# PacificBiosciences/ccs

Measured on AMD Instinct MI355X. Metric: ZMWs/sec (HiFi reads/sec), 10-pass x 10 kb synthetic, higher is better.
Workload: dtype f32

## Files before the change

### ccs_amd/csrc/ccsx_api.cpp

```cpp
#include <hip/hip_runtime.h>

#include <algorithm>
#include <cmath>
#include <cstdio>
#include <cstdlib>
#include <cstring>
#include <initializer_list>
#include <mutex>
#include <string>
#include <vector>

#include "ccsx.h"
#include "ccsx_internal.h"
#include "ccsx_kernels.h"
#include "refine_core.h"

#define HIPTRY(expr)                                                                                           \
    do {                                                                                                       \
        hipError_t e_ = (expr);                                                                                \
        if (e_ != hipSuccess) {                                                                                \
            ccsx_set_error(std::string(#expr) + ": " + hipGetErrorString(e_));                                 \
            return -2;                                                                                         \
        }                                                                                                      \
    } while (0)
// ... 1410 lines not shown
}
int ccsx_submit_hd_requests(ccsx_handle h, const ccsx_batch *b, ccsx_results *res, const ccsx_requests *rq, const ccsx_hd_request *hd, ccsx_ticket *ticket)
{
    Wants W;
    if (hd_requests_wants(rq, hd, b, __func__, &W)) return -1;
    return submit_impl(h, b, res, ticket, CCSX_RUN_FUSED, nullptr, nullptr, 0, W, __func__);
}
int ccsx_submit_hd(ccsx_handle h, const ccsx_batch *b, ccsx_results *res, const ccsx_extras *ex, const ccsx_hd_request *hd, ccsx_ticket *ticket)
{
    const ccsx_requests rq = {ex, nullptr, nullptr, nullptr, nullptr, {nullptr, nullptr, nullptr}};
    Wants W;
    if (hd_requests_wants(&rq, hd, b, __func__, &W)) return -1;
    return submit_impl(h, b, res, ticket, CCSX_RUN_FUSED, nullptr, nullptr, 0, W, __func__);
}
int ccsx_submit_handoff(ccsx_handle h, const ccsx_batch *b, ccsx_results *res, const ccsx_requests *rq, const ccsx_handoff_request *ho, ccsx_ticket *ticket)
{
    Wants W;
    if (requests_wants(rq, b, __func__, &W, ho) || (!ho && refuse(__func__, "null handoff request"))) return -1;
    return submit_impl(h, b, res, ticket, CCSX_RUN_FUSED, nullptr, nullptr, 0, W, __func__);
}
int ccsx_submit_barcodes(ccsx_handle h, const ccsx_batch *b, ccsx_results *res, const ccsx_requests *rq, const ccsx_barcode_request *bc, ccsx_ticket *ticket)
{
    Wants W;
    if ((!bc && refuse(__func__, "null barcode request")) || (!b && refuse(__func__, "null argument")) || requests_wants(rq, b, __func__, &W, nullptr, bc)) return -1;
    return submit_impl(h, b, res, ticket, CCSX_RUN_FUSED, nullptr, nullptr, 0, W, __func__);
}
static int represent_wants(ccsx_handle h, const ccsx_batch *b, const ccsx_requests *rq, const ccsx_represent_request *rp, const char *fn, Wants *W)
{
    if (!rp) return refuse(fn, "null represent request");
    if (!h || !b) return refuse(fn, "null argument");
    if (ccsx_represent_check(rp, b, &h->opts, fn)) return -1;
    if (rq && rq->coverage && rq->coverage->gate != 0) return refuse(fn, "the represent request is not combined with the coverage gate");
    if (requests_wants(rq, b, fn, W)) return -1;
    W->represent_req = *rp; W->represent = true;
    return 0;
}
int ccsx_submit_represent(ccsx_handle h, const ccsx_batch *b, ccsx_results *res, const ccsx_requests *rq, const ccsx_represent_request *rp, ccsx_ticket *ticket)
{
    Wants W;
    if (represent_wants(h, b, rq, rp, __func__, &W)) return -1;
    return submit_impl(h, b, res, ticket, CCSX_RUN_FUSED, nullptr, nullptr, 0, W, __func__);
}
int ccsx_submit_draft(ccsx_handle h, const ccsx_batch *b, ccsx_drafts *drafts, ccsx_ticket *ticket)
{
    return submit_impl(h, b, nullptr, ticket, CCSX_RUN_DRAFT, drafts, nullptr, 0, Wants{}, __func__);
}
int ccsx_submit_polish(ccsx_handle h, const ccsx_batch *b, const ccsx_drafts *drafts, ccsx_results *res, uint32_t flags, ccsx_ticket *ticket)
{
    return submit_impl(h, b, res, ticket, CCSX_RUN_POLISH, nullptr, drafts, flags, Wants{}, __func__);
}
int ccsx_draft_batch(ccsx_handle h, const ccsx_batch *b, ccsx_drafts *drafts)
{
    ccsx_ticket t;
    if (int rc = ccsx_submit_draft(h, b, drafts, &t)) return rc;
    return ccsx_wait(h, t);
}
int ccsx_polish_batch(ccsx_handle h, const ccsx_batch *b, const ccsx_drafts *drafts, ccsx_results *res, uint32_t flags)
{
    ccsx_ticket t;
    if (int rc = ccsx_submit_polish(h, b, drafts, res, flags, &t)) return rc;
    return ccsx_wait(h, t);
}

int ccsx_submit_refine(ccsx_handle h, const ccsx_batch *b, const ccsx_results *base, const int32_t *backbone, const ccsx_refine_tiles *tiles, ccsx_results *res,
                       ccsx_refine_report *report, ccsx_ticket *ticket)
{
    RefineReq rf;
    if (refine_request_check(b, base, backbone, tiles, report, &rf, __func__)) return -1;
    return submit_impl(h, b, res, ticket, CCSX_RUN_POLISH, nullptr, nullptr, CCSX_QV_ONLY, Wants{}, __func__, &rf);
}
int ccsx_refine_batch(ccsx_handle h, const ccsx_batch *b, const ccsx_results *base, const int32_t *backbone, const ccsx_refine_tiles *tiles, ccsx_results *res,
                      ccsx_refine_report *report)
{
    ccsx_ticket t;
    if (int rc = ccsx_submit_refine(h, b, base, backbone, tiles, res, report, &t)) return rc;
    return ccsx_wait(h, t);
}

static Slot *slot_of(ccsx_handle h, ccsx_ticket t)
{
    if (!h || t < 0) return nullptr;
    Slot &S = h->slot[t % CCSX_SLOTS];
    return S.ticket == t ? &S : nullptr;
}

int ccsx_wait(ccsx_handle h, ccsx_ticket ticket)
{
    Slot *S = slot_of(h, ticket);
    if (!S) { ccsx_set_error("ccsx_wait: unknown or recycled ticket"); return -1; }
    HIPTRY(hipSetDevice(h->device));
    return retire(h, *S);
}

int ccsx_poll(ccsx_handle h, ccsx_ticket ticket)
{
    Slot *S = slot_of(h, ticket);
    if (!S) { ccsx_set_error("ccsx_poll: unknown or recycled ticket"); return -1; }
    const hipError_t e = hipEventQuery(S->ev_done);
    if (e == hipErrorNotReady) return 0;
    if (e != hipSuccess) { ccsx_set_error(std::string("ccsx_poll: ") + hipGetErrorString(e)); return -2; }
    HIPTRY(hipSetDevice(h->device));
    return retire(h, *S) ? -2 : 1;
}

int ccsx_ticket_timings(ccsx_handle h, ccsx_ticket ticket, ccsx_timings *t)
{
    Slot *S = slot_of(h, ticket);
    if (!S || !t || !(S->ran || S->tm_ok)) { ccsx_set_error("ccsx_ticket_timings: unknown ticket"); return -1; }
    if (S->tm_ok) { *t = S->tm; return 0; }
    HIPTRY(hipSetDevice(h->device));
    return slot_timings(h, *S, t);
}

static int upload_impl(ccsx_handle h, const ccsx_batch *b, const Wants &W)
{
    if (!h) { ccsx_set_error("ccsx_upload: null handle"); return -1; }
    HIPTRY(hipSetDevice(h->device));
    for (auto &S : h->slot) if (int rc = retire(h, S)) return rc;
    Slot &S = h->slot[0];
    S.ticket = -1;
    const int rc = stage(h, S, b, h->s_comp, W);
    if (rc) { S.staged = false; return rc; }
    S.mode = CCSX_RUN_FUSED;
    HIPTRY(hipStreamSynchronize(h->s_comp));
    h->last = 0;
    return 0;
}

int ccsx_upload(ccsx_handle h, const ccsx_batch *b) { return upload_impl(h, b, Wants{}); }

int ccsx_run(ccsx_handle h)
{
    if (!h || !h->slot[0].staged || h->slot[0].mode != CCSX_RUN_FUSED) { ccsx_set_error("ccsx_run: no batch uploaded for the fused path: call ccsx_upload first"); return -1; }
    HIPTRY(hipSetDevice(h->device));
    h->last = 0;
    return launch(h, h->slot[0]);
}

int ccsx_sync(ccsx_handle h)
{
    if (!h) return -1;
    HIPTRY(hipSetDevice(h->device));
    HIPTRY(hipStreamSynchronize(h->s_draft));
    HIPTRY(hipStreamSynchronize(h->s_comp));
    Slot &S = h->slot[h->last];
#ifdef CCSX_PROFILE_PHASES
    if (S.staged && S.ran) {
        unsigned long long ph[16];
        HIPTRY(hipMemcpy(ph, S.P.phase, sizeof(ph), hipMemcpyDeviceToHost));
        static const char *nm[8] = {"prologue", "tables+lanes", "chunk plan", "fill", "score", "select/apply", "qv+store", "validity+list"};
        unsigned long long tot = 0;
        for (int i = 0; i < 8; ++i) tot += ph[i];
        for (int i = 0; i < 8; ++i) std::fprintf(stderr, "[ccsx phase] %-14s %6.2f %%  (%llu cycles)\n", nm[i], tot ? 100.0 * ph[i] / tot : 0.0, ph[i]);
        static const char *pn[6] = {"thr setup+read", "thr traceback", "thr ids+zero", "thr records", "thr order", "thr col records"};
        unsigned long long pt = 0;
        for (int i = 8; i < 14; ++i) pt += ph[i];
        for (int i = 8; i < 14; ++i) std::fprintf(stderr, "[ccsx phase] %-14s %6.2f %%  (%llu cycles)\n", pn[i - 8], pt ? 100.0 * ph[i] / pt : 0.0, ph[i]);
    }
#endif
#ifdef CCSX_DEBUG_CHECKS
    if (S.staged) {
        int32_t dbg[2] = {0, 0};
        HIPTRY(hipMemcpy(dbg, S.P.debug, 8, hipMemcpyDeviceToHost));
        if (dbg[0]) { ccsx_set_error("device bounds check failed: code " + std::to_string(dbg[0]) + " at kernel line " + std::to_string(dbg[1])); return -3; }
    }
#endif
    (void)S;
    return 0;
}

int ccsx_download(ccsx_handle h, ccsx_results *res)
{
    if (!h || !h->slot[0].ran || h->slot[0].mode != CCSX_RUN_FUSED || !res) { ccsx_set_error("ccsx_download: nothing to download: ccsx_upload + ccsx_run first"); return -1; }
    Slot &S = h->slot[0];
    if (int rc = check_results(S, res, S.P.out_kin != nullptr)) return rc;
    HIPTRY(hipSetDevice(h->device));
    if (int rc = enqueue_download(S, res, h->s_comp)) return rc;
    HIPTRY(hipStreamSynchronize(h->s_comp));
    finish_outputs(S, res, nullptr);
    return 0;
}

int ccsx_consensus_batch(ccsx_handle h, const ccsx_batch *b, ccsx_results *res)
{
    int rc;
    if ((rc = ccsx_upload(h, b))) return rc;
    if ((rc = ccsx_run(h))) return rc;
    if ((rc = ccsx_sync(h))) return rc;
    return ccsx_download(h, res);
}

int ccsx_pileup_rule_version(void) { return 1; }

static int consensus_sync(ccsx_handle h, const ccsx_batch *b, ccsx_results *res, const Wants &W, const char *fn)
{
    if (!h || !b || !res) return refuse(fn, "null argument");
    int rc;
    if ((rc = upload_impl(h, b, W))) return rc;
    Slot &S = h->slot[0];
    if ((rc = check_results(S, res, S.P.out_kin != nullptr)) || (rc = attach(h, S, W, h->s_comp))) return rc;
    HIPTRY(hipStreamSynchronize(h->s_comp));
    if ((rc = ccsx_run(h)) || (rc = ccsx_sync(h)) || (rc = ccsx_download(h, res))) return rc;
    if ((rc = enqueue_wants_download(S, W, h->s_comp))) return rc;
    HIPTRY(hipStreamSynchronize(h->s_comp));
    return 0;
}

int ccsx_consensus_pileup(ccsx_handle h, const ccsx_batch *b, ccsx_results *res, ccsx_pileup *pile)
{
    const ccsx_extras ex = {pile, nullptr, 0, 0};
    Wants W;
    if (build_wants(&ex, nullptr, nullptr, nullptr, nullptr, b, __func__, &W) || (!pile && refuse(__func__, "null argument"))) return -1;
    return consensus_sync(h, b, res, W, __func__);
}

int ccsx_tandem_rule_version(void) { return 1; }

int ccsx_consensus_extras(ccsx_handle h, const ccsx_batch *b, ccsx_results *res, const ccsx_extras *ex)
{
    Wants W;
    if (build_wants(ex, nullptr, nullptr, nullptr, nullptr, b, __func__, &W)) return -1;
    return consensus_sync(h, b, res, W, __func__);
}

int ccsx_consensus_hd_requests(ccsx_handle h, const ccsx_batch *b, ccsx_results *res, const ccsx_requests *rq, const ccsx_hd_request *hd)
{
    Wants W;
    if (hd_requests_wants(rq, hd, b, __func__, &W)) return -1;
    return consensus_sync(h, b, res, W, __func__);
}

int ccsx_consensus_hd(ccsx_handle h, const ccsx_batch *b, ccsx_results *res, const ccsx_extras *ex, const ccsx_hd_request *hd)
{
    const ccsx_requests rq = {ex, nullptr, nullptr, nullptr, nullptr, {nullptr, nullptr, nullptr}};
    Wants W;
    if (hd_requests_wants(&rq, hd, b, __func__, &W)) return -1;
    return consensus_sync(h, b, res, W, __func__);
}

void ccsx_fold_opts_default(ccsx_fold_opts *o)
{
    if (!o) return;
    o->max_occ = 8; o->min_hits = 12; o->min_arm = 200; o->min_span_tenths = 8; o->end_slack = 100;
}

int ccsx_fold_rule_version(void) { return 1; }

int ccsx_consensus_fold(ccsx_handle h, const ccsx_batch *b, ccsx_results *res, const ccsx_extras *ex, const ccsx_fold_request *fold)
{
    Wants W;
    if (build_wants(ex, nullptr, fold, nullptr, nullptr, b, __func__, &W) || (!fold && refuse(__func__, "null request or report"))) return -1;
    return consensus_sync(h, b, res, W, __func__);
}

void ccsx_adapter_opts_default(ccsx_adapter_opts *o)
{
    if (!o) return;
    o->max_dist_pct = 20; o->min_copies = 2; o->max_insert = 100; o->end_slack = 200;
}

int ccsx_adapter_rule_version(void) { return 1; }

int ccsx_adapter_set_default(ccsx_adapter_set *s)
{
    if (!s) { ccsx_set_error("ccsx_adapter_set_default: null argument"); return -1; }
    static const char hairpin[] = "ATCTCTCTCTTTTCCTCCTCCTCCGTTGTTGTTGTTGAGAGAGAT";
    std::memset(s, 0, sizeof *s);
    s->n_adapters = 1; s->len[0] = (int32_t)(sizeof hairpin - 1);
    for (int i = 0; i < s->len[0]; ++i) s->seq[0][i] = (uint8_t)(hairpin[i] == 'A' ? 0 : hairpin[i] == 'C' ? 1 : hairpin[i] == 'G' ? 2 : 3);
    return 0;
}

int ccsx_consensus_screen(ccsx_handle h, const ccsx_batch *b, ccsx_results *res, const ccsx_extras *ex, const ccsx_fold_request *fold, const ccsx_adapter_request *adapters)
{
    Wants W;
    if (build_wants(ex, nullptr, fold, adapters, nullptr, b, __func__, &W)) return -1;
    return consensus_sync(h, b, res, W, __func__);
}

void ccsx_control_opts_default(ccsx_control_opts *o)
{
    if (!o) return;
    o->max_occ = 4; o->min_matched = 30; o->min_ctl_tenths = 5; o->min_draft_tenths = 8;
}

int ccsx_control_rule_version(void) { return 1; }

int ccsx_consensus_control(ccsx_handle h, const ccsx_batch *b, ccsx_results *res, const ccsx_extras *ex, const ccsx_fold_request *fold, const ccsx_adapter_request *adapters,
                           const ccsx_control_request *control)
{
    Wants W;
    if (build_wants(ex, nullptr, fold, adapters, control, b, __func__, &W)) return -1;
    return consensus_sync(h, b, res, W, __func__);
}

void ccsx_coverage_opts_default(ccsx_coverage_opts *o)
{
    if (!o) return;
    o->drop_percent = 50; o->block = 30; o->min_spans = 0; o->max_lost_percent = 50;
}

int ccsx_coverage_rule_version(void) { return 1; }

int ccsx_consensus_requests(ccsx_handle h, const ccsx_batch *b, ccsx_results *res, const ccsx_requests *rq)
{
    Wants W;
    if (requests_wants(rq, b, __func__, &W)) return -1;
    return consensus_sync(h, b, res, W, __func__);
}

// ... 378 lines not shown
```

### ccs_amd/csrc/ccsx_kernels.hip

```cpp
#include <hip/hip_runtime.h>
#include <stdint.h>
#include <cstdio>
#include <cstdlib>

#include "ccsx.h"
#include "ccsx_kernels.h"
#include "wave_ops.h"

#define LANDED(x) asm volatile("" : "+v"(x))

#if (defined(CCSX_EXP_NO_FILL) || defined(CCSX_EXP_NO_SCORE) || defined(CCSX_EXP_ONE_ROUND) || defined(CCSX_EXP_ALL_VALID) || defined(CCSX_EXP_CHEAP_VALIDITY) || \
     defined(CCSX_EXP_NO_ROWS) || defined(CCSX_EXP_NO_SCORE_LOG) || defined(CCSX_EXP_SKIP_ROUND2_SCORE) || defined(CCSX_EXP_NO_QV_EXP) || defined(CCSX_EXP_REPEAT) || defined(CCSX_EXP_NO_BANDMASK) || \
     defined(CCSX_EXP_HOT_PROLOGUE) || defined(CCSX_EXIT_AFTER_PROLOGUE)) && !defined(CCSX_EXPERIMENT)
#error "CCSX_EXP_* / CCSX_EXIT_AFTER_PROLOGUE switches produce wrong results: build them with -DCCSX_EXPERIMENT (never ship such a library)"
#endif
#define CCSX_STR2(x) #x
#define CCSX_STR(x) CCSX_STR2(x)
int ccsx_kernel_is_experiment()
{
#ifdef CCSX_EXPERIMENT
    return 1;
#else
    return 0;
#endif
// ... 599 lines not shown
        const int vb = rec.x & 3;
        const int p0 = rec.y;
        const unsigned long long multim = actm & M_NE0(rec.x & 0xe00);
        const unsigned long long far0m = actm & M_NE0(rec.x & CREC_FAR0);
        const uint32_t slot0 = p0 < 0 ? PRING : (uint32_t)(p0 & (PRING - 1));
        int k0x, k0y, k0z;
        { const uint32_t ka = kinBase + slot0 * 16; k0x = LDS_I32(ka); k0y = LDS_I32(ka + 4); k0z = LDS_I32(ka + 8); }
        if (__builtin_expect(far0m != 0ull, 0)) { if (rec.x & CREC_FAR0) { const int4 t = kinfo[p0]; k0x = t.x; k0y = t.y; k0z = t.z; } LANDED(k0x); LANDED(k0y); LANDED(k0z); }
        int ulo = k0x, ubr = k0z;
        int plo1 = 0, plo2 = 0;
        if (multim) {
            const int np = (rec.x >> 8) & 15;
            const bool act = live && k < n0;
            int bestcm = k0y;
            for (int q = 1; q < CCSX_MAXPRED; ++q) {
                if ((actm & M_SGT(np, q)) == 0ull) break;
                int pq = q == 1 ? rec.z : rec.w;
                if (q >= 3) {
                    if (act && np > q) pq = pxw[(size_t)k * 4 + (q - 3)];
                    LANDED(pq);
                }
                const bool on = act && np > q;
                const bool farq = on && k - pq > PRING;
                const uint32_t ka = kinBase + (on ? (uint32_t)(pq & (PRING - 1)) : (uint32_t)PRING) * 16;
                int qx = LDS_I32(ka), qy = LDS_I32(ka + 4), qz = LDS_I32(ka + 8);
                if (__builtin_expect(M_NE0(farq ? 1 : 0) != 0ull, 0)) { if (farq) { const int4 t = kinfo[pq]; qx = t.x; qy = t.y; qz = t.z; } LANDED(qx); LANDED(qy); LANDED(qz); }
                if (q == 1) plo1 = qx; else if (q == 2) plo2 = qx;
                if (on && qy > bestcm) { bestcm = qy; ulo = qx; ubr = qz; }
            }
        }
        int lo = imed3(ubr + (1 - PB / 2), ulo, ulo + 2);
        lo = lo < hiI ? lo : hiI;
        lo = lo > 0 ? lo : 0;
        if (__builtin_expect((actm & M_UGT(lo - c0, CH16 - PB - 2)) != 0ull, 0)) {
            __syncthreads();
            if (live && k < n0 && (unsigned)(lo - c0) > (unsigned)(CH16 - PB - 2)) {
                c0 = lo - 128 > 0 ? lo - 128 : 0;
                load_read_chunk_m1(sRead[gq], rb, I, rev, c0, l);
            }
            __syncthreads();
        }
        const int r0w = lo + l2;
        int s0, s1;
        {
            const uint32_t idx = (uint32_t)(r0w - c0) & (CH16 - 1);
            const uint32_t wa = readBase + ((idx >> 4) << 2);
            const uint32_t wlo = (uint32_t)LDS_I32(wa), whi = (uint32_t)LDS_I32(wa + 4);
            const uint32_t t = __builtin_amdgcn_alignbit(whi, wlo, (idx & 15u) << 1);
            s0 = (vb == (int)(t & 3u)) ? SC_MATCH : SC_MISMATCH;
            s1 = (vb == (int)((t >> 2) & 3u)) ? SC_MATCH : SC_MISMATCH;
        }
        int b0, b1, m0, m1;
        {
            const int w = imed3(r0w - k0x + 3, 1, PGS - 3);
            const uint32_t src = ringBase + slot0 * (PGS * 4) + ((uint32_t)w << 2);
            int x0 = LDS_I32(src), y0 = LDS_I32(src + 4), y1 = LDS_I32(src + 8);
            if (__builtin_expect(far0m != 0ull, 0)) {
                if (rec.x & CREC_FAR0) {
                    const int32_t *Mu = Mcol + (size_t)p0 * PB;
                    const int o = r0w - k0x - 1;
                    x0 = (unsigned)o < (unsigned)PB ? Mu[o] : NEGV;
                    y0 = (unsigned)(o + 1) < (unsigned)PB ? Mu[o + 1] : NEGV;
                    y1 = (unsigned)(o + 2) < (unsigned)PB ? Mu[o + 2] : NEGV;
                }
                LANDED(x0); LANDED(y0); LANDED(y1);
            }
            const int d0 = x0 + s0, e0 = y0 + SC_DEL, d1 = y0 + s1, e1 = y1 + SC_DEL;
            const bool t0 = e0 > d0, t1 = e1 > d1;
            b0 = t0 ? e0 : d0; m0 = t0 ? 1 : 0;
            b1 = t1 ? e1 : d1; m1 = t1 ? 1 : 0;
        }
        if (multim) {
            const int np = (rec.x >> 8) & 15;
            const bool act = live && k < n0;
            for (int q = 1; q < CCSX_MAXPRED; ++q) {
                if ((actm & M_SGT(np, q)) == 0ull) break;
                const bool on = act && np > q;
                int pq = q == 1 ? rec.z : rec.w, plo = q == 1 ? plo1 : plo2;
                if (q >= 3) {
                    if (on) {
                        pq = pxw[(size_t)k * 4 + (q - 3)];
                        if (k - pq > PRING) plo = kinfo[pq].x; else plo = LDS_I32(kinBase + (uint32_t)(pq & (PRING - 1)) * 16);
                    }
                    LANDED(pq); LANDED(plo);
                }
                const bool farq = on && k - pq > PRING;
                const int off = r0w - plo;
                const int w = imed3(off + 3, 1, PGS - 3);
                const uint32_t src = ringBase + (on ? (uint32_t)(pq & (PRING - 1)) : (uint32_t)PRING) * (PGS * 4) + ((uint32_t)w << 2);
                int x0 = LDS_I32(src), y0 = LDS_I32(src + 4), y1 = LDS_I32(src + 8);
                if (__builtin_expect(M_NE0(farq ? 1 : 0) != 0ull, 0)) {
                    if (farq) {
                        const int32_t *Mu = Mcol + (size_t)pq * PB;
                        const int o = off - 1;
                        x0 = (unsigned)o < (unsigned)PB ? Mu[o] : NEGV;
                        y0 = (unsigned)(o + 1) < (unsigned)PB ? Mu[o + 1] : NEGV;
                        y1 = (unsigned)(o + 2) < (unsigned)PB ? Mu[o + 2] : NEGV;
                    }
                    LANDED(x0); LANDED(y0); LANDED(y1);
                }
                const int mq = q << 1;
                int c;
                c = x0 + s0;     if (on && c > b0) { b0 = c; m0 = mq; }
                c = y0 + SC_DEL; if (on && c > b0) { b0 = c; m0 = mq | 1; }
                c = y0 + s1;     if (on && c > b1) { b1 = c; m1 = mq; }
                c = y1 + SC_DEL; if (on && c > b1) { b1 = c; m1 = mq | 1; }
            }
        }
        { const int c = b0 + SC_INS; if (c > b1) { b1 = c; m1 = 15; } }
        {
            const int S = row_scan_max_i32(b1 + l8);
            const int Sp = __builtin_amdgcn_update_dpp(-(1 << 30), S, DPP_ROW_SHR(1), 0xf, 0xf, false);
            const int c0v = Sp - (l8 - 8 - SC_INS);
            const int c1v = Sp - (l8 - 8 - 2 * SC_INS);
            if (c0v > b0) { b0 = c0v; m0 = 15; }
            if (c1v > b1) { b1 = c1v; m1 = 15; }
        }
        if (r0w > I || b0 < NEGV / 2) b0 = NEGV;
        if (r0w >= I || b1 < NEGV / 2) b1 = NEGV;
        int cm, br;
        {
            const int f = -(1 << 24);
            const int k0_ = ((b0 > f ? b0 : f) * 64) | kRow0, k1_ = ((b1 > f ? b1 : f) * 64) | kRow1;
            const int key = row_allmax_i32(k0_ > k1_ ? k0_ : k1_);
            cm = key >> 6; br = (lo + 63) - (key & 63);
        }
        if (__builtin_expect((actm & M_SGT(lo + PB, I)) != 0ull, 0)) {
            const int e = r0w == I ? b0 : (r0w + 1 == I ? b1 : NEGV);
            const int ev = __builtin_amdgcn_ds_bpermute(bcastAddr, row_scan_max_i32(e));
            if (live && k < n0 && ev > NEGV / 2 && ev > bs) { bs = ev; kend = k; }
        }
        if (live && k < n0) {
            *(int2 *)&sRing[gq][k & (PRING - 1)][4 + l2] = make_int2(b0, b1);
            *mvp = (uint8_t)(m0 | (m1 << 4));
            if (l == 0) {
                sKin[gq][k & (PRING - 1)] = make_int4(lo, cm, br, 0);
                *lop = lo;
            }
            if (__builtin_expect((rec.x & CREC_NEED) != 0, 0)) {
                *(int2 *)Mp = make_int2(b0, b1);
                if (l == 0) *kip = make_int4(lo, cm, br, p0);
            }
        }
    }
#undef M_NE0
#undef M_SLT
#undef M_SGT
#undef M_UGT
#undef LDS_I32
    __threadfence_block();
    if (live && l == 0) { st[ST_KEND] = kend; st[ST_BS] = bs; }
}

__global__ __launch_bounds__(64) __attribute__((amdgpu_waves_per_eu(8, 8))) void k_poa_thread(KParams P, int z0, int pass, int rr, int b0)
{
    const int bx = (int)blockIdx.x + b0;
    __shared__ __attribute__((aligned(16))) uint8_t sMv[TB_BLOCK * POA_MV_BYTES];
    const int lane = threadIdx.x;
    uint32_t *sread = dyn_lds;
    PoaSlot g = poa_slot(P, bx);
    if (z0 + bx >= P.n_zmw) return;
    if (!g.st[ST_LIVE] || !g.st[ST_OK] || rr >= g.st[ST_NPOA]) return;
    TPH_T0();
    const int z = rfl(P.zmw_perm[z0 + bx]);
    const int r0 = rfl(P.read_off[z]);
    const int bb = rfl(g.st[ST_BB]), nreads = rfl(g.st[ST_NREADS]), npoa = rfl(g.st[ST_NPOA]);
    const int r = r0 + (bb + rr < nreads ? bb + rr : bb + rr - nreads);
    const uint8_t *rb = P.bases + P.base_off[r];
    const int I = rfl((int)(P.base_off[r + 1] - P.base_off[r]));
    const int kend = rfl(g.st[ST_KEND]), bsc = rfl(g.st[ST_BS]);
    int32_t *const plog = (P.poa_log && pass < 2 && rr < P.poa_log_stride) ? P.poa_log + ((size_t)(2 * z + pass) * P.poa_log_stride + rr) * CCSX_POA_LOG_WORDS : nullptr;
    auto log_pass = [&](int threaded, int nv) { if (plog && lane == 0) { plog[0] = I; plog[1] = bsc; plog[2] = kend; plog[3] = threaded; plog[4] = nv; } };
    if (kend < 0 || bsc < I) { log_pass(0, g.st[ST_N]); return; }
    const int rev = rfl(((P.flags[r] & 1) != g.st[ST_REV0]) ? 1 : 0);
    const int vcap = rfl(P.vcap[z]);
    const int n0 = rfl(g.st[ST_N]);
    const int par = rfl(g.st[ST_PAR]);
    const int4 *crec = par ? g.crec1 : g.crec0, *pxc = par ? g.px1 : g.px0;
    int4 *crec_nx = par ? g.crec0 : g.crec1, *px_nx = par ? g.px0 : g.px1;
    load_read_packed(sread, rb, I, rev, lane);
    __syncthreads();
    TPH(8);
    {
        int k = kend, i = I;
        int4 kiN = make_int4(0, 0, 0, -1), crN = make_int4(0, -1, -1, -1);
        int kbN = -1;
        uint4 mvN0 = make_uint4(0, 0, 0, 0);
        auto fetch = [&](int kb_) {
            const int kk = kb_ + lane;
            kbN = kb_;
            kiN = make_int4(0, 0, 0, -1); crN = make_int4(0, -1, -1, -1);
            if (kb_ >= 0) {
                if (kk < n0) { crN = crec[kk]; kiN = make_int4(g.loK[kk], 0, 0, crN.y); }
                mvN0 = ((const uint4 *)(g.mvK + (size_t)kb_ * POA_MV_BYTES))[lane];
            }
        };
        fetch((k / TB_BLOCK) * TB_BLOCK);
        while (k >= 0) {
            const int kb = (k / TB_BLOCK) * TB_BLOCK;
            if (kbN != kb) fetch(kb);
            __syncthreads();
            const int4 kiL = kiN, crL = crN;
            const int metaL = crN.x;
            ((uint4 *)sMv)[lane] = mvN0;
            fetch(kb - TB_BLOCK);
            __syncthreads();
            while (k >= kb) {
                int kl = k - kb;
                int mknown;
                {
                    const int kls = kl - lane;
                    const int src = kls & 63;
                    const int lo_s = __shfl(kiL.x, src), pp_s = __shfl(kiL.w, src);
                    const int off = i - lane - lo_s;
                    const bool inb = kls >= 0 && i - lane >= 1 && (unsigned)off < (unsigned)PB;
                    const int m_s = inb ? ((sMv[kls * POA_MV_BYTES + (off >> 1)] >> ((off & 1) << 2)) & 15) : 255;
                    const unsigned long long simple = __ballot(m_s == 0 && pp_s == k - lane - 1);
                    const int R = (simple == ~0ull) ? 64 : __ffsll((long long)~simple) - 1;
                    if (R > 0) {
                        const int meta_s = __shfl(metaL, src);
                        if (lane < R) {
                            const int ir = i - lane - 1;
                            g.pathv[ir] = ((meta_s & 3) == read_base_packed(sread, ir)) ? k - lane : -1;
                        }
                        k -= R; i -= R;
                        if (R >= 64 || k < kb) continue;
                        kl = k - kb;
                    }
                    mknown = rl(m_s, R);
                }
                const int lo_k = rl(kiL.x, kl);
                CHK(i - lo_k >= 0 && i - lo_k < PB && i >= 0, 101);
                const int mo = i - lo_k;
                const int m = mknown != 255 ? mknown : rfl((sMv[kl * POA_MV_BYTES + (mo >> 1)] >> ((mo & 1) << 2)) & 15);
                const int t = m == 15 ? MV_INS : (m & 1), slot = m >> 1;
                CHK(i >= 1 || t == MV_DEL, 102);
                if (t == MV_INS) { if (lane == 0) g.pathv[i - 1] = -1; --i; continue; }
                const int meta = rl(metaL, kl);
                const int np = (meta >> 8) & 15;
                int up;
                if (np == 0) up = -1;
                else if (slot == 0) up = rl(kiL.w, kl);
                else if (slot == 1) up = rl(crL.z, kl);
                else if (slot == 2) up = rl(crL.w, kl);
                else up = rfl(((const int32_t *)pxc)[(size_t)k * 4 + (slot - 3)]);
                if (t == MV_DIAG) {
                    if (lane == 0) g.pathv[i - 1] = ((meta & 3) == read_base_packed(sread, i - 1)) ? k : -1;
                    --i;
                }
                CHK(up < k && up >= -1, 103);
                k = up;
            }
            k = rfl(k); i = rfl(i);
        }
        for (int q = lane; q < i; q += LANES) g.pathv[q] = -1;
    }
    __threadfence_block();
    TPH(9);
    int32_t *cnt = g.bestK;
    auto newpos = [&](int q) -> int { return q + cnt[q]; };
    for (int q = lane; q <= n0; q += LANES) { cnt[q] = 0; g.onpK[q] = 0; }
    __threadfence_block();
    TPH(10);
    int lastEx = -1, nnew = 0;
    for (int c0 = 0; c0 < I; c0 += 2 * LANES) {
        int w[2], wn[2], ex[2];
        bool valid[2], isnew[2], lastOfRun[2];
#pragma unroll
        for (int u = 0; u < 2; ++u) {
            const int i = c0 + u * LANES + lane;
            valid[u] = i < I;
            const int ic = valid[u] ? i : I - 1;
            w[u] = g.pathv[ic];
            wn[u] = g.pathv[ic + 1 < I ? ic + 1 : ic];
        }
#pragma unroll
        for (int u = 0; u < 2; ++u) {
            const int i = c0 + u * LANES + lane;
            isnew[u] = valid[u] && w[u] < 0;
            nnew += __popcll(__ballot(isnew[u]));
            const int incl = wave_scan_max_i32((valid[u] && !isnew[u]) ? i : -1);
            int e = wave_shr1_i32(incl, -1);
            e = e > lastEx ? e : lastEx;
            ex[u] = e;
            const int li = rl(incl, 63);
            lastEx = li > lastEx ? li : lastEx;
            lastOfRun[u] = isnew[u] && ((i + 1 >= I) || (wn[u] >= 0));
        }
        int av[2];
#pragma unroll
        for (int u = 0; u < 2; ++u) av[u] = g.pathv[(lastOfRun[u] && ex[u] >= 0) ? ex[u] : 0];
#pragma unroll
        for (int u = 0; u < 2; ++u) {
            const int i = c0 + u * LANES + lane;
            if (valid[u] && !isnew[u]) g.onpK[w[u]] = 1;
            if (lastOfRun[u]) {
                const int ap = ex[u] >= 0 ? av[u] : -1;
                CHK(ap >= -1 && ap < n0, 106);
                cnt[ap + 1] = i - ex[u];
            }
        }
    }
    nnew = rfl(nnew);
    if (n0 + nnew > vcap) { if (lane == 0) g.st[ST_OK] = 0; log_pass(0, n0); return; }
    __threadfence_block();
    TPH(11);
    int carry = 0;
    for (int c0 = 0; c0 <= n0; c0 += 4 * LANES) {
        int cv[4];
#pragma unroll
        for (int u = 0; u < 4; ++u) { const int q = c0 + u * LANES + lane; cv[u] = cnt[q <= n0 ? q : n0]; }
#pragma unroll
        for (int u = 0; u < 4; ++u) {
            const int q = c0 + u * LANES + lane;
            const int incl = wave_scan_add_i32(q <= n0 ? cv[u] : 0);
            if (q <= n0) cnt[q] = carry + incl;
            carry += rl(incl, 63);
        }
    }
    const int n = n0 + nnew;
    for (int q = lane; q < n; q += LANES) g.needK[q] = 0;
    __threadfence_block();
    auto carry_over = [&](int q, int kn, int4 rec, int4 &pxr) -> int4 {
        const int np = (rec.x >> 8) & 15;
        rec.x &= ~CREC_FAR0;
        if (np > 0) { rec.y = newpos(rec.y); if (kn - rec.y > PRING) { g.needK[rec.y] = 1; rec.x |= CREC_FAR0; } }
        if (np > 1) { rec.z = newpos(rec.z); if (kn - rec.z > PRING) g.needK[rec.z] = 1; }
        if (np > 2) { rec.w = newpos(rec.w); if (kn - rec.w > PRING) g.needK[rec.w] = 1; }
        if (np > 3) {
            pxr = pxc[q];
            for (int e = 3; e < np; ++e) { const int pn = newpos(int4_get(pxr, e - 3)); int4_set(pxr, e - 3, pn); if (kn - pn > PRING) g.needK[pn] = 1; }
        }
        return rec;
    };
    for (int q0 = 0; q0 < n0; q0 += 2 * LANES) {
        int4 rec[2]; int kn[2]; bool go[2];
#pragma unroll
        for (int u = 0; u < 2; ++u) {
            const int q = q0 + u * LANES + lane;
            go[u] = q < n0 && !g.onpK[q < n0 ? q : 0];
            rec[u] = make_int4(0, -1, -1, -1); kn[u] = 0;
            if (go[u]) { rec[u] = crec[q]; kn[u] = newpos(q); }
        }
#pragma unroll
        for (int u = 0; u < 2; ++u) if (go[u]) {
            const int q = q0 + u * LANES + lane;
            int4 pxr = make_int4(-1, -1, -1, -1);
            const int4 r = carry_over(q, kn[u], rec[u], pxr);
            CHK(kn[u] >= 0 && kn[u] < n, 105);
            crec_nx[kn[u]] = r;
            if (((r.x >> 8) & 15) > 3) px_nx[kn[u]] = pxr;
        }
    }
    TPH(12);
    lastEx = -1;
    int prevP = -1;
    for (int c0 = 0; c0 < I; c0 += LANES) {
        const int i = c0 + lane;
        const bool valid = i < I;
        const int w = g.pathv[valid ? i : I - 1];
        const bool isnew = valid && w < 0;
        const int incl = wave_scan_max_i32((valid && !isnew) ? i : -1);
        int ex = wave_shr1_i32(incl, -1);
        ex = ex > lastEx ? ex : lastEx;
        { const int li = rl(incl, 63); lastEx = li > lastEx ? li : lastEx; }
        const int av = g.pathv[(isnew && ex >= 0) ? ex : 0];
        int4 rec = make_int4(0, -1, -1, -1);
        if (valid && !isnew) rec = crec[w];
        const int qa = valid ? (isnew ? (ex >= 0 ? av : 0) : w) : 0;
        int P = newpos(qa);
        if (isnew) P = (ex >= 0 ? P + 1 : 0) + (i - ex - 1);
        if (!valid) P = -1;
        int Pp = wave_shr1_i32(P, prevP);
        prevP = rl(P, 63);
        if (valid) {
            CHK(P >= 0 && P < n, 104);
            int4 pxr = make_int4(-1, -1, -1, -1);
            bool pxdirty = false;
            if (isnew) rec = make_int4(read_base_packed(sread, i) | ((Pp >= 0 ? 1 : 0) << 8) | (1 << CREC_NREADS_SHIFT), Pp, -1, -1);
            else {
                rec = carry_over(w, P, rec, pxr);
                rec.x += 1 << CREC_NREADS_SHIFT;
                if (Pp >= 0) {
                    const int np = (rec.x >> 8) & 15;
                    bool found = false;
                    if (np > 0) found |= rec.y == Pp;
                    if (np > 1) found |= rec.z == Pp;
                    if (np > 2) found |= rec.w == Pp;
                    for (int e = 3; e < np; ++e) found |= int4_get(pxr, e - 3) == Pp;
                    if (!found && np < CCSX_MAXPRED) {
                        if (np == 0) rec.y = Pp; else if (np == 1) rec.z = Pp; else if (np == 2) rec.w = Pp; else { int4_set(pxr, np - 3, Pp); pxdirty = true; }
                        rec.x += 1 << 8;
                        if (P - Pp > PRING) { g.needK[Pp] = 1; if (np == 0) rec.x |= CREC_FAR0; }
                    }
                }
            }
            crec_nx[P] = rec;
            if (((rec.x >> 8) & 15) > 3 || pxdirty) px_nx[P] = pxr;
        }
    }
    __threadfence_block();
    if (lane == 0) { g.st[ST_N] = n; g.st[ST_NADDED] += 1; g.st[ST_PAR] ^= 1; }
    log_pass(1, n);
    (void)npoa;
    TPH(13);
}

__global__ __launch_bounds__(64) __attribute__((amdgpu_waves_per_eu(8, 8))) void k_poa_finish(KParams P, int z0, int pass, int b0)
{
    const int bx = (int)blockIdx.x + b0;
    const int lane = threadIdx.x;
    PoaSlot g = poa_slot(P, bx);
    if (z0 + bx >= P.n_zmw) return;
    if (!g.st[ST_LIVE]) return;
    const int z = rfl(P.zmw_perm[z0 + bx]);
    const int ok = rfl(g.st[ST_OK]), n = rfl(g.st[ST_N]), nadded = rfl(g.st[ST_NADDED]);
    const int4 *crec = g.st[ST_PAR] ? g.crec1 : g.crec0;
    const int32_t *pxw = (const int32_t *)(g.st[ST_PAR] ? g.px1 : g.px0);
    int Ld = 0, nw = 0, stat = -1;
    if (ok && n > 0) {
        int kbest = -1, sb = NEGV, best_prev = 0;
        for (int kb = 0; kb < n; kb += LANES) {
            const int kkL = kb + lane;
            int4 cL = make_int4(0, -1, -1, -1);
            if (kkL < n) cL = crec[kkL];
            const int nblk = (n - kb) < LANES ? (n - kb) : LANES;
            const int npL = (cL.x >> 8) & 15;
            const int wL = kkL < n ? 2 * ((cL.x >> CREC_NREADS_SHIFT) & 127) - nadded : 0;
            const int Pw = wave_scan_add_i32(wL);
            const bool headL = kkL < n && (lane == 0 || npL != 1 || cL.y != kkL - 1);
            unsigned long long heads = __ballot(headL);
            const unsigned long long headmask = heads;
            int hb = 0, bpv = kkL - 1;
            while (heads) {
                const int j = (int)__ffsll((long long)heads) - 1;
                heads &= heads - 1;
                const int k = kb + j;
                const int np = rl(npL, j);
                int b = 0, p = -1;
                for (int q = 0; q < np; ++q) {
                    int pu;
                    if (q < 3) pu = q == 0 ? rl(cL.y, j) : (q == 1 ? rl(cL.z, j) : rl(cL.w, j));
                    else pu = rfl(pxw[(size_t)k * 4 + (q - 3)]);
                    CHK(pu >= 0 && pu < k, 108);
                    int bu;
                    if (pu >= kb) {
                        const int pj = pu - kb;
                        const int hd = 63 - __clzll((long long)(headmask & ((2ull << pj) - 1ull)));
                        bu = rl(hb, hd) + rl(Pw, pj) - rl(Pw, hd);
                    } else bu = pu == kb - 1 ? best_prev : rfl(g.bestK[pu]);
                    if (bu > b) { b = bu; p = pu; }
                }
                const int bv = b + rl(wL, j);
                if (lane == j) { hb = bv; bpv = p; }
            }
            const int hdL = 63 - __clzll((long long)(headmask & ((2ull << lane) - 1ull)));
            int myBest = __shfl(hb, hdL) + Pw - __shfl(Pw, hdL);
            const unsigned long long nonpos = __ballot(kkL < n && myBest <= 0);
            if ((nonpos << 1) & ~headmask & (nblk == 64 ? ~0ull : (1ull << nblk) - 1ull)) {
                int myBp = -1; myBest = 0;
                int bprev = best_prev;
                for (int j = 0; j < nblk; ++j) {
                    const int k = kb + j;
                    const int np = rl(npL, j);
                    int b = 0, p = -1;
                    for (int q = 0; q < np; ++q) {
                        int pu;
                        if (q < 3) pu = q == 0 ? rl(cL.y, j) : (q == 1 ? rl(cL.z, j) : rl(cL.w, j));
                        else pu = rfl(pxw[(size_t)k * 4 + (q - 3)]);
                        const int bu = pu == k - 1 ? bprev : ((pu >= kb) ? rl(myBest, pu - kb) : rfl(g.bestK[pu]));
                        if (bu > b) { b = bu; p = pu; }
                    }
                    const int bv = b + rl(wL, j);
                    if (lane == j) { myBest = bv; myBp = p; }
                    bprev = bv;
                }
                bpv = myBp;
            }
            if (kkL < n) { g.bestK[kkL] = myBest; g.bpK[kkL] = bpv; }
            const int key = wave_max_i32(kkL < n ? myBest * 64 + (63 - lane) : INT32_MIN);
            const int bmax = key >> 6;
            if (bmax > sb) { sb = bmax; kbest = kb + 63 - (key & 63); }
            best_prev = rl(myBest, nblk - 1);
            __threadfence_block();
        }
        uint8_t *tmp = (uint8_t *)g.pathv;
        int len = 0, k = kbest;
        while (k >= 0) {
            const int kb = (k >> 6) << 6;
            const int kk = kb + lane;
            const int bpL = kk < n ? g.bpK[kk] : -1;
            const int bL = kk < n ? (crec[kk].x & 255) : 0;
            const unsigned long long chain = __ballot(kk < n && bpL == kk - 1);
            while (k >= kb) {
                const int kl = k - kb;
                const unsigned long long inv = ~chain & ((2ull << kl) - 1ull);
                const int t = inv ? 63 - __clzll((long long)inv) : 0;
                CHK(len + kl - t < n, 107);
                if (lane >= t && lane <= kl) tmp[len + (kl - lane)] = (uint8_t)bL;
                len += kl - t + 1;
                k = inv ? rl(bpL, t) : kb - 1;
            }
        }
        __threadfence_block();
        if (len <= P.dcap[z]) {
            uint8_t *draft = P.draft + P.seq_off[z];
            for (int q = lane; q < len; q += LANES) draft[q] = tmp[len - 1 - q];
            Ld = len;
        }
        __threadfence_block();
    }
    if (Ld <= 0) stat = CCSX_DRAFT_FAILURE;
    else if (Ld < P.opts.min_length) stat = CCSX_TOO_SHORT;
    else if (Ld > P.opts.max_length) stat = CCSX_TOO_LONG;
    else {
        nw = poa_windows(P, z, Ld, lane);
    }
    if (lane == 0) { P.draft_len[z] = Ld; P.nwin[z] = (stat < 0) ? nw : 0; P.zstat[z] = (stat < 0) ? CCSX_SUCCESS : stat; }
}

__device__ __forceinline__ int need_col(const int32_t *wb, int nw, int Ld, int k)
{
    return k == 0 ? 0 : (k == 2 * nw - 1 ? Ld : wb[(k + 1) >> 1] + ((k & 1) ? -CCSX_WIN_OVERHANG : CCSX_WIN_OVERHANG));
}
struct AlignEnd { int M, O, lo; unsigned K; };
template <int REV>
__device__ __forceinline__ AlignEnd align_pass(const KParams &P, const uint32_t *sread, int I, const uint8_t *d, int Ld, const int32_t *wb, int nw,
                                               int32_t *Osave, int lane)
{
    const int nneed = 2 * nw;
    int32_t *lo_need = Osave + (size_t)P.need_max * 128;
    int32_t *cm_need = lo_need + P.need_max + 64, *br_need = cm_need + P.need_max, *eb_need = br_need + P.need_max;
    int2 *OMsave = (int2 *)Osave;
    int kk = 1;
    auto need_at = [&](int k) { return REV ? Ld - need_col(wb, nw, Ld, nneed - 1 - k) : need_col(wb, nw, Ld, k); };
    int next_need = rfl(need_at(1));
    int Mprev = (lane <= I) ? lane * SC_INS : NEGV;
    int Oprev = 0;
    unsigned Kprev = (lane >= 1) ? 1u : 0u;
    int ecol = 0;
    int lo = 0, br = 0;
    int rbv = (lane >= 1 && lane <= I) ? read_base_packed(sread, lane - 1) : 4;
    const int hiI = I - (CCSX_BAND - 1) > 0 ? I - (CCSX_BAND - 1) : 0;
    BaseCursor bcur; bcur.w0 = 0; bcur.vw = 0u;
    const int nwords = (I + 15) >> 4;
    for (int jb = 0; jb < Ld; jb += LANES) {
        const int dL = (jb + lane < Ld) ? d[REV ? Ld - 1 - (jb + lane) : jb + lane] : 0;
        cursor_load(bcur, sread, nwords, lo + 61, lane);
        asm volatile("" :: "v"(dL), "v"(bcur.vw));
        const int nblk = (Ld - jb) < LANES ? (Ld - jb) : LANES;
        auto column = [&](const int jj) {
// ... 3442 lines not shown
```

Before: 41410.

## Pack on-path flag into shift words and software-pipeline POA graph renumbering loops

Merges the separate onpK flag array and the cnt shift array into one 32-bit word per node, with the top bit as the on-path flag, so each node needs one load instead of two. It clears needK with packed 32-bit stores fused into the zeroing loop and drops the later needK clear. The anchor node is now found with a wave max-scan instead of a dependent pathv lookup. The off-path and path loops gain unroll factors with next-iteration prefetch of shift words and pathv, and predecessor shifts are batched ahead of use. The extra scans and the higher unroll raise register pressure and subtly change which nodes get the on-path flag, with some correctness risk.

```diff
diff --git a/ccs_amd/csrc/ccsx_api.cpp b/ccs_amd/csrc/ccsx_api.cpp
--- a/ccs_amd/csrc/ccsx_api.cpp
+++ b/ccs_amd/csrc/ccsx_api.cpp
@@ -1586,10 +1586,10 @@
         unsigned long long tot = 0;
         for (int i = 0; i < 8; ++i) tot += ph[i];
         for (int i = 0; i < 8; ++i) std::fprintf(stderr, "[ccsx phase] %-14s %6.2f %%  (%llu cycles)\n", nm[i], tot ? 100.0 * ph[i] / tot : 0.0, ph[i]);
-        static const char *pn[6] = {"thr setup+read", "thr traceback", "thr ids+zero", "thr records", "thr order", "thr col records"};
+        static const char *pn[7] = {"thr setup+read", "thr traceback", "thr zero", "thr A runs", "thr C off-path", "thr D path", "thr B prefix"};
         unsigned long long pt = 0;
-        for (int i = 8; i < 14; ++i) pt += ph[i];
-        for (int i = 8; i < 14; ++i) std::fprintf(stderr, "[ccsx phase] %-14s %6.2f %%  (%llu cycles)\n", pn[i - 8], pt ? 100.0 * ph[i] / pt : 0.0, ph[i]);
+        for (int i = 8; i < 15; ++i) pt += ph[i];
+        for (int i = 8; i < 15; ++i) std::fprintf(stderr, "[ccsx phase] %-14s %6.2f %%  (%llu cycles)\n", pn[i - 8], pt ? 100.0 * ph[i] / pt : 0.0, ph[i]);
     }
 #endif
 #ifdef CCSX_DEBUG_CHECKS
diff --git a/ccs_amd/csrc/ccsx_kernels.hip b/ccs_amd/csrc/ccsx_kernels.hip
--- a/ccs_amd/csrc/ccsx_kernels.hip
+++ b/ccs_amd/csrc/ccsx_kernels.hip
@@ -775,6 +775,7 @@
     if (live && l == 0) { st[ST_KEND] = kend; st[ST_BS] = bs; }
 }
 
+constexpr int THR_AU = 2, THR_BU = 4, THR_CU = 4, THR_DU = 2;
 __global__ __launch_bounds__(64) __attribute__((amdgpu_waves_per_eu(8, 8))) void k_poa_thread(KParams P, int z0, int pass, int rr, int b0)
 {
     const int bx = (int)blockIdx.x + b0;
@@ -880,48 +881,42 @@
     }
     __threadfence_block();
     TPH(9);
-    int32_t *cnt = g.bestK;
-    auto newpos = [&](int q) -> int { return q + cnt[q]; };
-    for (int q = lane; q <= n0; q += LANES) { cnt[q] = 0; g.onpK[q] = 0; }
+    uint32_t *cw = (uint32_t *)g.bestK;
+    constexpr uint32_t CW_ONP = 0x80000000u, CW_S = 0x7fffffffu;
+    {
+        const int nz = n0 + I < vcap ? n0 + I : vcap;
+        const int nkw = (nz + 3) >> 2, top = nkw > n0 + 1 ? nkw : n0 + 1;
+        uint32_t *nk = (uint32_t *)g.needK;
+        for (int q = lane; q < top; q += LANES) { if (q <= n0) cw[q] = 0; if (q < nkw) nk[q] = 0; }
+    }
     __threadfence_block();
     TPH(10);
-    int lastEx = -1, nnew = 0;
-    for (int c0 = 0; c0 < I; c0 += 2 * LANES) {
-        int w[2], wn[2], ex[2];
-        bool valid[2], isnew[2], lastOfRun[2];
-#pragma unroll
-        for (int u = 0; u < 2; ++u) {
+    int lastEx = -1, lastW = -1, nnew = 0;
+    for (int c0 = 0; c0 < I; c0 += THR_AU * LANES) {
+        int w[THR_AU], wn[THR_AU];
+#pragma unroll
+        for (int u = 0; u < THR_AU; ++u) {
             const int i = c0 + u * LANES + lane;
-            valid[u] = i < I;
-            const int ic = valid[u] ? i : I - 1;
+            const int ic = i < I ? i : I - 1;
             w[u] = g.pathv[ic];
             wn[u] = g.pathv[ic + 1 < I ? ic + 1 : ic];
         }
 #pragma unroll
-        for (int u = 0; u < 2; ++u) {
+        for (int u = 0; u < THR_AU; ++u) {
             const int i = c0 + u * LANES + lane;
-            isnew[u] = valid[u] && w[u] < 0;
-            nnew += __popcll(__ballot(isnew[u]));
-            const int incl = wave_scan_max_i32((valid[u] && !isnew[u]) ? i : -1);
-            int e = wave_shr1_i32(incl, -1);
-            e = e > lastEx ? e : lastEx;
-            ex[u] = e;
-            const int li = rl(incl, 63);
-            lastEx = li > lastEx ? li : lastEx;
-            lastOfRun[u] = isnew[u] && ((i + 1 >= I) || (wn[u] >= 0));
-        }
-        int av[2];
-#pragma unroll
-        for (int u = 0; u < 2; ++u) av[u] = g.pathv[(lastOfRun[u] && ex[u] >= 0) ? ex[u] : 0];
-#pragma unroll
-        for (int u = 0; u < 2; ++u) {
-            const int i = c0 + u * LANES + lane;
-            if (valid[u] && !isnew[u]) g.onpK[w[u]] = 1;
-            if (lastOfRun[u]) {
-                const int ap = ex[u] >= 0 ? av[u] : -1;
-                CHK(ap >= -1 && ap < n0, 106);
-                cnt[ap + 1] = i - ex[u];
-            }
+            const bool valid = i < I, isnew = valid && w[u] < 0, exist = valid && w[u] >= 0;
+            nnew += __popcll(__ballot(isnew));
+            const int inclI = wave_scan_max_i32(exist ? i : -1), inclW = wave_scan_max_i32(exist ? w[u] : -1);
+            int ex = wave_shr1_i32(inclI, -1), ap = wave_shr1_i32(inclW, -1);
+            ex = ex > lastEx ? ex : lastEx;
+            ap = ap > lastW ? ap : lastW;
+            { const int li = rl(inclI, 63), lw = rl(inclW, 63); lastEx = li > lastEx ? li : lastEx; lastW = lw > lastW ? lw : lastW; }
+            if (isnew) {
+                if (i + 1 >= I || wn[u] >= 0) {
+                    CHK(ap >= -1 && ap < n0, 106);
+                    cw[ap + 1] = (uint32_t)(i - ex) | ((i + 1 < I && wn[u] == ap + 1) ? CW_ONP : 0u);
+                }
+            } else if (exist && (ex == i - 1 || ap + 1 != w[u])) cw[w[u]] = CW_ONP;
         }
     }
     nnew = rfl(nnew);
@@ -929,97 +924,129 @@
     __threadfence_block();
     TPH(11);
     int carry = 0;
-    for (int c0 = 0; c0 <= n0; c0 += 4 * LANES) {
-        int cv[4];
-#pragma unroll
-        for (int u = 0; u < 4; ++u) { const int q = c0 + u * LANES + lane; cv[u] = cnt[q <= n0 ? q : n0]; }
-#pragma unroll
-        for (int u = 0; u < 4; ++u) {
+    for (int c0 = 0; c0 <= n0; c0 += THR_BU * LANES) {
+        int cv[THR_BU];
+#pragma unroll
+        for (int u = 0; u < THR_BU; ++u) { const int q = c0 + u * LANES + lane; cv[u] = (int)cw[q <= n0 ? q : n0]; }
+#pragma unroll
+        for (int u = 0; u < THR_BU; ++u) {
             const int q = c0 + u * LANES + lane;
-            const int incl = wave_scan_add_i32(q <= n0 ? cv[u] : 0);
-            if (q <= n0) cnt[q] = carry + incl;
+            const int incl = wave_scan_add_i32(q <= n0 ? (int)((uint32_t)cv[u] & CW_S) : 0);
+            if (q <= n0) cw[q] = ((uint32_t)cv[u] & CW_ONP) | (uint32_t)(carry + incl);
             carry += rl(incl, 63);
         }
     }
     const int n = n0 + nnew;
-    for (int q = lane; q < n; q += LANES) g.needK[q] = 0;
     __threadfence_block();
-    auto carry_over = [&](int q, int kn, int4 rec, int4 &pxr) -> int4 {
+    TPH(14);
+    auto shift_of = [&](int p) -> int { return (int)(cw[p > 0 ? p : 0] & CW_S); };
+    auto carry_over = [&](int q, int kn, int4 rec, int sy, int sz, int sw, int4 &pxr) -> int4 {
         const int np = (rec.x >> 8) & 15;
         rec.x &= ~CREC_FAR0;
-        if (np > 0) { rec.y = newpos(rec.y); if (kn - rec.y > PRING) { g.needK[rec.y] = 1; rec.x |= CREC_FAR0; } }
-        if (np > 1) { rec.z = newpos(rec.z); if (kn - rec.z > PRING) g.needK[rec.z] = 1; }
-        if (np > 2) { rec.w = newpos(rec.w); if (kn - rec.w > PRING) g.needK[rec.w] = 1; }
+        if (np > 0) { rec.y += sy; if (kn - rec.y > PRING) { g.needK[rec.y] = 1; rec.x |= CREC_FAR0; } }
+        if (np > 1) { rec.z += sz; if (kn - rec.z > PRING) g.needK[rec.z] = 1; }
+        if (np > 2) { rec.w += sw; if (kn - rec.w > PRING) g.needK[rec.w] = 1; }
         if (np > 3) {
             pxr = pxc[q];
-            for (int e = 3; e < np; ++e) { const int pn = newpos(int4_get(pxr, e - 3)); int4_set(pxr, e - 3, pn); if (kn - pn > PRING) g.needK[pn] = 1; }
+            for (int e = 3; e < np; ++e) { const int p = int4_get(pxr, e - 3), pn = p + shift_of(p); int4_set(pxr, e - 3, pn); if (kn - pn > PRING) g.needK[pn] = 1; }
         }
         return rec;
     };
-    for (int q0 = 0; q0 < n0; q0 += 2 * LANES) {
-        int4 rec[2]; int kn[2]; bool go[2];
-#pragma unroll
-        for (int u = 0; u < 2; ++u) {
+    uint32_t wvn[THR_CU];
+#pragma unroll
+    for (int u = 0; u < THR_CU; ++u) { const int q = u * LANES + lane; wvn[u] = cw[q < n0 ? q : n0]; }
+    for (int q0 = 0; q0 < n0; q0 += THR_CU * LANES) {
+        int4 rec[THR_CU]; uint32_t wv[THR_CU];
+        int sy[THR_CU], sz[THR_CU], sw[THR_CU];
+#pragma unroll
+        for (int u = 0; u < THR_CU; ++u) { wv[u] = wvn[u]; const int q = q0 + (THR_CU + u) * LANES + lane; wvn[u] = cw[q < n0 ? q : n0]; }
+#pragma unroll
+        for (int u = 0; u < THR_CU; ++u) {
             const int q = q0 + u * LANES + lane;
-            go[u] = q < n0 && !g.onpK[q < n0 ? q : 0];
-            rec[u] = make_int4(0, -1, -1, -1); kn[u] = 0;
-            if (go[u]) { rec[u] = crec[q]; kn[u] = newpos(q); }
-        }
-#pragma unroll
-        for (int u = 0; u < 2; ++u) if (go[u]) {
+            rec[u] = make_int4(0, -1, -1, -1);
+            if (q < n0 && !(wv[u] & CW_ONP)) rec[u] = crec[q];
+        }
+#pragma unroll
+        for (int u = 0; u < THR_CU; ++u) {
             const int q = q0 + u * LANES + lane;
-            int4 pxr = make_int4(-1, -1, -1, -1);
-            const int4 r = carry_over(q, kn[u], rec[u], pxr);
-            CHK(kn[u] >= 0 && kn[u] < n, 105);
-            crec_nx[kn[u]] = r;
-            if (((r.x >> 8) & 15) > 3) px_nx[kn[u]] = pxr;
+            sy[u] = sz[u] = sw[u] = 0;
+            if (q < n0 && !(wv[u] & CW_ONP)) { sy[u] = shift_of(rec[u].y); sz[u] = shift_of(rec[u].z); sw[u] = shift_of(rec[u].w); }
+        }
+#pragma unroll
+        for (int u = 0; u < THR_CU; ++u) {
+            const int q = q0 + u * LANES + lane;
+            if (q < n0 && !(wv[u] & CW_ONP)) {
+                const int kn = q + (int)(wv[u] & CW_S);
+                int4 pxr = make_int4(-1, -1, -1, -1);
+                const int4 r = carry_over(q, kn, rec[u], sy[u], sz[u], sw[u], pxr);
+                CHK(kn >= 0 && kn < n, 105);
+                crec_nx[kn] = r;
+                if (((r.x >> 8) & 15) > 3) px_nx[kn] = pxr;
+            }
         }
     }
     TPH(12);
-    lastEx = -1;
+    lastEx = -1; lastW = -1;
     int prevP = -1;
-    for (int c0 = 0; c0 < I; c0 += LANES) {
-        const int i = c0 + lane;
-        const bool valid = i < I;
-        const int w = g.pathv[valid ? i : I - 1];
-        const bool isnew = valid && w < 0;
-        const int incl = wave_scan_max_i32((valid && !isnew) ? i : -1);
-        int ex = wave_shr1_i32(incl, -1);
-        ex = ex > lastEx ? ex : lastEx;
-        { const int li = rl(incl, 63); lastEx = li > lastEx ? li : lastEx; }
-        const int av = g.pathv[(isnew && ex >= 0) ? ex : 0];
-        int4 rec = make_int4(0, -1, -1, -1);
-        if (valid && !isnew) rec = crec[w];
-        const int qa = valid ? (isnew ? (ex >= 0 ? av : 0) : w) : 0;
-        int P = newpos(qa);
-        if (isnew) P = (ex >= 0 ? P + 1 : 0) + (i - ex - 1);
-        if (!valid) P = -1;
-        int Pp = wave_shr1_i32(P, prevP);
-        prevP = rl(P, 63);
-        if (valid) {
-            CHK(P >= 0 && P < n, 104);
-            int4 pxr = make_int4(-1, -1, -1, -1);
-            bool pxdirty = false;
-            if (isnew) rec = make_int4(read_base_packed(sread, i) | ((Pp >= 0 ? 1 : 0) << 8) | (1 << CREC_NREADS_SHIFT), Pp, -1, -1);
-            else {
-                rec = carry_over(w, P, rec, pxr);
-                rec.x += 1 << CREC_NREADS_SHIFT;
-                if (Pp >= 0) {
-                    const int np = (rec.x >> 8) & 15;
-                    bool found = false;
-                    if (np > 0) found |= rec.y == Pp;
-                    if (np > 1) found |= rec.z == Pp;
-                    if (np > 2) found |= rec.w == Pp;
-                    for (int e = 3; e < np; ++e) found |= int4_get(pxr, e - 3) == Pp;
-                    if (!found && np < CCSX_MAXPRED) {
-                        if (np == 0) rec.y = Pp; else if (np == 1) rec.z = Pp; else if (np == 2) rec.w = Pp; else { int4_set(pxr, np - 3, Pp); pxdirty = true; }
-                        rec.x += 1 << 8;
-                        if (P - Pp > PRING) { g.needK[Pp] = 1; if (np == 0) rec.x |= CREC_FAR0; }
+    int wnx[THR_DU];
+#pragma unroll
+    for (int u = 0; u < THR_DU; ++u) { const int i = u * LANES + lane; wnx[u] = g.pathv[i < I ? i : I - 1]; }
+    for (int c0 = 0; c0 < I; c0 += THR_DU * LANES) {
+        int w[THR_DU], ex[THR_DU], qa[THR_DU], sy[THR_DU], sz[THR_DU], sw[THR_DU];
+        int4 rcv[THR_DU]; uint32_t wq[THR_DU];
+#pragma unroll
+        for (int u = 0; u < THR_DU; ++u) { w[u] = wnx[u]; const int i = c0 + (THR_DU + u) * LANES + lane; wnx[u] = g.pathv[i < I ? i : I - 1]; }
+#pragma unroll
+        for (int u = 0; u < THR_DU; ++u) {
+            const int i = c0 + u * LANES + lane;
+            const bool valid = i < I, exist = valid && w[u] >= 0;
+            const int inclI = wave_scan_max_i32(exist ? i : -1), inclW = wave_scan_max_i32(exist ? w[u] : -1);
+            int e = wave_shr1_i32(inclI, -1), ap = wave_shr1_i32(inclW, -1);
+            e = e > lastEx ? e : lastEx;
+            ap = ap > lastW ? ap : lastW;
+            { const int li = rl(inclI, 63), lw = rl(inclW, 63); lastEx = li > lastEx ? li : lastEx; lastW = lw > lastW ? lw : lastW; }
+            ex[u] = e;
+            qa[u] = valid ? (exist ? w[u] : (ap > 0 ? ap : 0)) : 0;
+            rcv[u] = crec[exist ? w[u] : 0];
+            wq[u] = cw[qa[u]];
+        }
+#pragma unroll
+        for (int u = 0; u < THR_DU; ++u) { sy[u] = shift_of(rcv[u].y); sz[u] = shift_of(rcv[u].z); sw[u] = shift_of(rcv[u].w); }
+#pragma unroll
+        for (int u = 0; u < THR_DU; ++u) {
+            const int i = c0 + u * LANES + lane;
+            const bool valid = i < I, isnew = valid && w[u] < 0;
+            int P = qa[u] + (int)(wq[u] & CW_S);
+            if (isnew) P = (ex[u] >= 0 ? P + 1 : 0) + (i - ex[u] - 1);
+            if (!valid) P = -1;
+            int Pp = wave_shr1_i32(P, prevP);
+            prevP = rl(P, 63);
+            if (valid) {
+                CHK(P >= 0 && P < n, 104);
+                int4 pxr = make_int4(-1, -1, -1, -1);
+                bool pxdirty = false;
+                int4 rec;
+                if (isnew) rec = make_int4(read_base_packed(sread, i) | ((Pp >= 0 ? 1 : 0) << 8) | (1 << CREC_NREADS_SHIFT), Pp, -1, -1);
+                else {
+                    rec = carry_over(w[u], P, rcv[u], sy[u], sz[u], sw[u], pxr);
+                    rec.x += 1 << CREC_NREADS_SHIFT;
+                    if (Pp >= 0) {
+                        const int np = (rec.x >> 8) & 15;
+                        bool found = false;
+                        if (np > 0) found |= rec.y == Pp;
+                        if (np > 1) found |= rec.z == Pp;
+                        if (np > 2) found |= rec.w == Pp;
+                        for (int e = 3; e < np; ++e) found |= int4_get(pxr, e - 3) == Pp;
+                        if (!found && np < CCSX_MAXPRED) {
+                            if (np == 0) rec.y = Pp; else if (np == 1) rec.z = Pp; else if (np == 2) rec.w = Pp; else { int4_set(pxr, np - 3, Pp); pxdirty = true; }
+                            rec.x += 1 << 8;
+                            if (P - Pp > PRING) { g.needK[Pp] = 1; if (np == 0) rec.x |= CREC_FAR0; }
+                        }
                     }
                 }
-            }
-            crec_nx[P] = rec;
-            if (((rec.x >> 8) & 15) > 3 || pxdirty) px_nx[P] = pxr;
+                crec_nx[P] = rec;
+                if (((rec.x >> 8) & 15) > 3 || pxdirty) px_nx[P] = pxr;
+            }
         }
     }
     __threadfence_block();
```

Result: no change. 41600, median of 6 (+0.5%).
